# ZackHodari/morgana

Hardware: AMD Instinct MI355X
Metric: acoustic frames/sec (fwd+bwd+step), F0Model 600->1, batch 256x1000 (higher is better)
Workload: dtype bf16

## Files before the change

### morgana_amd/csrc/gemm_bf16_big.hip

```cpp
#include "common.h"
#include "phone_front.h"
#include "expand_reduce.h"

#include <type_traits>

typedef __bf16 bfv8 __attribute__((ext_vector_type(8)));
typedef __bf16 bfv4 __attribute__((ext_vector_type(4)));


#define MG_ZERO_ELEMS 16384
__device__ uint16_t g_zero_row[MG_ZERO_ELEMS];

__device__ __forceinline__ void glds16(const uint16_t* src, unsigned char* lds_wave_base) {
    const unsigned lds_off = (unsigned)(unsigned long long)((__attribute__((address_space(3))) unsigned char*)lds_wave_base);
    const unsigned lds_uni = __builtin_amdgcn_readfirstlane(lds_off);
    unsigned keep;
    asm volatile("s_mov_b32 %0, m0\n\ts_mov_b32 m0, %2\n\ts_nop 0\n\tglobal_load_lds_dwordx4 %1, off\n\ts_mov_b32 m0, %0"
                 : "=&s"(keep)
                 : "v"(src), "s"(lds_uni)
                 : "memory");
}


#define WAIT_VM_BARRIER(N) asm volatile("s_waitcnt vmcnt(" #N ")\n\ts_barrier" ::: "memory")
#define WAIT_LGKM_BARRIER() asm volatile("s_waitcnt lgkmcnt(0)\n\ts_barrier" ::: "memory")

MG_STAMP_DECL(g_stamps_nt);

#define NT_BIG_LDS(BN_) (((BN_) == 256 ? 4 : 6) * (256 * 64 + (BN_) * 64))
template <int BN, int EPI, int X3 = 0>
__device__ __forceinline__ void gemm_nt_big_body(unsigned char* __restrict__ smem, const unsigned block_id, const uint16_t* __restrict__ A,
                                                 int lda, const int32_t* __restrict__ rows, int64_t M, int K, const uint16_t* __restrict__ Bm,
                                                 int ldb, int N, const float* __restrict__ bias_in, const uint16_t* __restrict__ H, int ldh,
                                                 const int32_t* __restrict__ h_rows, void* __restrict__ Cv_in, int ldc, int tiles_m, int tiles_n,
                                                 int c_f32, float* __restrict__ colsum = nullptr, int wt = 0) {
    const float* bias = bias_in;
    void* Cv = Cv_in;
    constexpr int BM = 256;
    constexpr int WAVES_N = BN / 64;
    constexpr int WAVES_M = 8 / WAVES_N;
    constexpr int WM = BM / WAVES_M;
    constexpr int TM = WM / 32, TN = 2;
    constexpr int A_BYTES = BM * 64, B_BYTES = BN * 64;
    constexpr int STAGE = A_BYTES + B_BYTES;
    constexpr int GA = BM / 16 / 8;
    constexpr int GB = BN / 16 / 8;
    constexpr int NL = GA + GB;
    constexpr int NS = (BN == 256) ? 4 : 6;

    static_assert(NS * STAGE == NT_BIG_LDS(BN), "LDS size helper");

    unsigned tile_id = block_id;
    int my_pass = 0;
    if (X3 == 2) {
        const unsigned per_pass = (unsigned)((tiles_m + 7) / 8) * 8u * (unsigned)tiles_n;
        my_pass = (int)(block_id / per_pass);
        tile_id = block_id - (unsigned)my_pass * per_pass;
    }
    const int xcd = tile_id & 7, jj = tile_id >> 3;
    const int tile_n = jj % tiles_n;
    const int tile_m = (jj / tiles_n) * 8 + xcd;
    if (tile_m >= tiles_m) return;

    const int tid = threadIdx.x, lane = tid & 63;
    const int wave = __builtin_amdgcn_readfirstlane(tid >> 6);
#ifdef MG_STAMPS
    unsigned long long ts0, ts1 = 0, ts2, ts3, tr0, tr1, ta, tb, sum_wait = 0, sum_issue = 0;
    MG_STAMP(ts0);
    MG_STAMP_REAL(tr0);
#endif
    const int wm0 = (wave / WAVES_N) * WM, wn0 = (wave % WAVES_N) * 64;
    const int64_t m0 = (int64_t)tile_m * BM;
    const int n0 = tile_n * BN;
    const int n_kp = (K + 31) / 32;
    const int n_kt = X3 == 1 ? 3 * n_kp : n_kp;
    const int a_lo = lda >> 1, b_lo = ldb >> 1;
    if (X3 == 2) {
        if (my_pass > 0) bias = nullptr;
        Cv = reinterpret_cast<float*>(Cv) + (size_t)my_pass * (size_t)M * ldc;
    }

    const uint16_t* asrc[GA];
    const uint16_t* bsrc[GB];
#pragma unroll
    for (int i = 0; i < GA; ++i) {
        const int row = (wave * GA + i) * 16 + (lane >> 2);
        const int c = (lane & 3) ^ ((row >> 2) & 3);
        const int64_t m = m0 + row;
        const uint16_t* p = g_zero_row;
        if (m < M) {
            if (rows) {
                const int r = rows[m];
                if (r >= 0) p = A + (size_t)r * lda;
            } else {
                p = A + (size_t)m * lda;
            }
        }
        asrc[i] = p + c * 8;
    }
#pragma unroll
    for (int i = 0; i < GB; ++i) {
        const int row = (wave * GB + i) * 16 + (lane >> 2);
        const int c = (lane & 3) ^ ((row >> 2) & 3);
        const int n = n0 + row;
        bsrc[i] = (n < N ? Bm + (size_t)n * ldb : g_zero_row) + c * 8;
    }

    auto issue = [&](int kt) {
        unsigned char* st = smem + (kt % NS) * STAGE;
        int ka = kt * 32, kb = kt * 32;
        if (X3) {
            const int pass = X3 == 2 ? my_pass : kt % 3, w = (X3 == 2 ? kt : kt / 3) * 32;
            ka = w + (pass == 2 ? a_lo : 0);
            kb = w + (pass == 1 ? b_lo : 0);
        }
#pragma unroll
        for (int i = 0; i < GA; ++i) glds16(asrc[i] + ka, st + (wave * GA + i) * 1024);
#pragma unroll
        for (int i = 0; i < GB; ++i) glds16(bsrc[i] + kb, st + A_BYTES + (wave * GB + i) * 1024);
    };

    f32x16 acc[TM][TN];
#pragma unroll
    for (int i = 0; i < TM; ++i)
#pragma unroll
        for (int j = 0; j < TN; ++j)
#pragma unroll
            for (int r = 0; r < 16; ++r) acc[i][j][r] = 0.f;

    const int lr = lane & 31, lh = lane >> 5;
    int aoff[TM], boff[TN];
#pragma unroll
    for (int i = 0; i < TM; ++i) {
        const int row = wm0 + i * 32 + lr;
        aoff[i] = row * 64 + ((lh ^ ((row >> 2) & 3)) << 4);
    }
#pragma unroll
    for (int j = 0; j < TN; ++j) {
        const int row = wn0 + j * 32 + lr;
        boff[j] = A_BYTES + row * 64 + ((lh ^ ((row >> 2) & 3)) << 4);
    }

#pragma unroll
    for (int p = 0; p < NS - 1; ++p)
        if (p < n_kt) issue(p);
    for (int kt = 0; kt < n_kt; ++kt) {
        MG_STAMP(ta);
        {
            const int fly = min(n_kt - 1 - kt, NS - 2);
            if (NL == 4) {
                if (fly >= 2) WAIT_VM_BARRIER(8); else if (fly == 1) WAIT_VM_BARRIER(4); else WAIT_VM_BARRIER(0);
            } else if (NS == 4) {
                if (fly >= 2) WAIT_VM_BARRIER(6); else if (fly == 1) WAIT_VM_BARRIER(3); else WAIT_VM_BARRIER(0);
            } else {
                if (fly >= 4) WAIT_VM_BARRIER(12); else if (fly == 3) WAIT_VM_BARRIER(9); else if (fly == 2) WAIT_VM_BARRIER(6);
                else if (fly == 1) WAIT_VM_BARRIER(3); else WAIT_VM_BARRIER(0);
            }
        }
        MG_STAMP(tb);
        MG_STAMP_ADD(sum_wait, tb, ta);
#ifdef MG_STAMPS
        if (kt == 0) ts1 = tb;
#endif
        if (kt + NS - 1 < n_kt) issue(kt + NS - 1);
        MG_STAMP(ta);
        MG_STAMP_ADD(sum_issue, ta, tb);
        const unsigned char* st = smem + (kt % NS) * STAGE;
#pragma unroll
        for (int ks = 0; ks < 2; ++ks) {
            bfv8 a[TM], b[TN];
#pragma unroll
            for (int i = 0; i < TM; ++i) a[i] = *reinterpret_cast<const bfv8*>(st + (aoff[i] ^ (ks << 5)));
#pragma unroll
            for (int j = 0; j < TN; ++j) b[j] = *reinterpret_cast<const bfv8*>(st + (boff[j] ^ (ks << 5)));
#pragma unroll
            for (int i = 0; i < TM; ++i)
#pragma unroll
                for (int j = 0; j < TN; ++j) {
                    if (EPI_IS_GRAD(EPI)) acc[i][j] = mg_mfma_32x32x16(a[i], b[j], acc[i][j]);
                    else acc[i][j] = mg_mfma_32x32x16(b[j], a[i], acc[i][j]);
                }
        }
    }

#ifdef MG_STAMPS
    MG_STAMP(ts2);
#endif
    if (EPI_IS_GRAD(EPI)) {
        constexpr int STG_LD = 68;
        WAIT_LGKM_BARRIER();
        float* stg = reinterpret_cast<float*>(smem) + wave * 32 * STG_LD;
        float csum[8];
#pragma unroll
        for (int e = 0; e < 8; ++e) csum[e] = 0.f;
#pragma unroll
        for (int i = 0; i < TM; ++i) {
#pragma unroll
            for (int j = 0; j < TN; ++j)
#pragma unroll
                for (int r = 0; r < 16; ++r) stg[((r & 3) + 8 * (r >> 2) + 4 * lh) * STG_LD + j * 32 + lr] = acc[i][j][r];
#pragma unroll
            for (int it = 0; it < 4; ++it) {
                const int rl = it * 8 + (lane >> 3);
                const int cl = (lane & 7) * 8;
                const int64_t row = m0 + wm0 + i * 32 + rl;
                const int col = n0 + wn0 + cl;
                const f32x4 v0 = *reinterpret_cast<const f32x4*>(&stg[rl * STG_LD + cl]);
                const f32x4 v1 = *reinterpret_cast<const f32x4*>(&stg[rl * STG_LD + cl + 4]);
                if (row >= M) continue;
                const int64_t hrow = h_rows ? (int64_t)h_rows[row] : row;
                const bfv8 hv = *reinterpret_cast<const bfv8*>(H + (size_t)hrow * ldh + col);
                float v[8] = {v0.x, v0.y, v0.z, v0.w, v1.x, v1.y, v1.z, v1.w};
                if (X3) {
                    const bfv8 hl = *reinterpret_cast<const bfv8*>(H + (size_t)hrow * ldh + (ldh >> 1) + col);
                    bfv8 o_hi, o_lo;
#pragma unroll
                    for (int e = 0; e < 8; ++e) {
#pragma clang fp contract(off)
                        const float h = (float)hv[e] + (float)hl[e];
                        const float x = v[e] * h * (1.f - h);
                        csum[e] += x;
                        o_hi[e] = (__bf16)x;
                        o_lo[e] = (__bf16)(x - (float)o_hi[e]);
                    }
                    uint16_t* crow = reinterpret_cast<uint16_t*>(Cv) + (size_t)row * ldc + col;
                    mg_store16_sel(wt, crow, __builtin_bit_cast(mg_u32x4, o_hi));
                    mg_store16_sel(wt, crow + (ldc >> 1), __builtin_bit_cast(mg_u32x4, o_lo));
                    continue;
                }
#pragma unroll
                for (int e = 0; e < 8; ++e) v[e] = mg_epi_dact<EPI>(v[e], (float)hv[e]);
                if (c_f32) {
                    float* crow = reinterpret_cast<float*>(Cv) + (size_t)row * ldc + col;
                    *reinterpret_cast<f32x4*>(crow) = f32x4{v[0], v[1], v[2], v[3]};
                    *reinterpret_cast<f32x4*>(crow + 4) = f32x4{v[4], v[5], v[6], v[7]};
                } else {
                    bfv8 o;
#pragma unroll
                    for (int e = 0; e < 8; ++e) o[e] = (__bf16)v[e];
                    mg_store16_sel(wt, reinterpret_cast<uint16_t*>(Cv) + (size_t)row * ldc + col, __builtin_bit_cast(mg_u32x4, o));
                }
            }
        }
        if (X3 && colsum) {
#pragma unroll
            for (int e = 0; e < 8; ++e) {
                csum[e] += __shfl_xor(csum[e], 8, 64);
                csum[e] += __shfl_xor(csum[e], 16, 64);
                csum[e] += __shfl_xor(csum[e], 32, 64);
            }
            if (lane < 8) {
                float* dst = colsum + ((size_t)tile_m * WAVES_M + (wave / WAVES_N)) * N + n0 + wn0 + lane * 8;
                *reinterpret_cast<f32x4*>(dst) = f32x4{csum[0], csum[1], csum[2], csum[3]};
                *reinterpret_cast<f32x4*>(dst + 4) = f32x4{csum[4], csum[5], csum[6], csum[7]};
            }
        }
        return;
    }

    float bv[TN][16];
    if (!EPI_IS_GRAD(EPI)) {
#pragma unroll
        for (int j = 0; j < TN; ++j)
#pragma unroll
            for (int g = 0; g < 4; ++g)
#pragma unroll
                for (int e = 0; e < 4; ++e) bv[j][4 * g + e] = bias ? bias[n0 + wn0 + j * 32 + 8 * g + 4 * lh + e] : 0.f;
    }
    if (!c_f32) {
        constexpr int SP = 144;
        WAIT_LGKM_BARRIER();
        unsigned char* patch = smem + wave * (32 * SP);
        const int prow = lane >> 3, pchunk = lane & 7;
#pragma unroll
        for (int i = 0; i < TM; ++i) {
#pragma unroll
            for (int j = 0; j < TN; ++j)
#pragma unroll
                for (int g = 0; g < 4; ++g) {
                    float v[4];
#pragma unroll
                    for (int e = 0; e < 4; ++e) {
                        float x = acc[i][j][4 * g + e] + bv[j][4 * g + e];
                        x = mg_epi_act<EPI, true>(x);
                        v[e] = x;
                    }
                    typedef __bf16 bfv2 __attribute__((ext_vector_type(2)));
                    typedef unsigned int u32x2_t __attribute__((ext_vector_type(2)));
                    const u32x2_t pk = u32x2_t{__builtin_bit_cast(unsigned int, bfv2{(__bf16)v[0], (__bf16)v[1]}),
                                               __builtin_bit_cast(unsigned int, bfv2{(__bf16)v[2], (__bf16)v[3]})};
                    *reinterpret_cast<u32x2_t*>(patch + lr * SP + (j * 32 + 8 * g + 4 * lh) * 2) = pk;
                }
#pragma unroll
            for (int it = 0; it < 4; ++it) {
                typedef unsigned int u32x4_t __attribute__((ext_vector_type(4)));
                const int rl = it * 8 + prow;
                const u32x4_t o = *reinterpret_cast<const u32x4_t*>(patch + rl * SP + pchunk * 16);
                const int64_t m = m0 + wm0 + i * 32 + rl;
                if (m < M) *reinterpret_cast<u32x4_t*>(reinterpret_cast<uint16_t*>(Cv) + (size_t)m * ldc + n0 + wn0 + pchunk * 8) = o;
            }
        }
    } else
#pragma unroll
    for (int i = 0; i < TM; ++i) {
        const int64_t m = m0 + wm0 + i * 32 + lr;
        const bool live = m < M;
#pragma unroll
        for (int j = 0; j < TN; ++j) {
            if (!live) continue;
            float* crow = reinterpret_cast<float*>(Cv) + (size_t)m * ldc + n0 + wn0 + j * 32 + 4 * lh;
#pragma unroll
            for (int g = 0; g < 4; ++g) {
                float v[4];
#pragma unroll
                for (int e = 0; e < 4; ++e) {
                    float x = acc[i][j][4 * g + e] + bv[j][4 * g + e];
                    x = mg_epi_act<EPI, true>(x);
                    v[e] = x;
                }
                *reinterpret_cast<f32x4*>(crow + 8 * g) = f32x4{v[0], v[1], v[2], v[3]};
            }
        }
    }
#ifdef MG_STAMPS
    asm volatile("s_waitcnt vmcnt(0)" ::: "memory");
    MG_STAMP(ts3);
    MG_STAMP_REAL(tr1);
    const int sb = block_id;
    MG_STAMP_STORE(g_stamps_nt, sb, wave, lane, 0, ts0);
    MG_STAMP_STORE(g_stamps_nt, sb, wave, lane, 1, ts1);
    MG_STAMP_STORE(g_stamps_nt, sb, wave, lane, 2, ts2);
    MG_STAMP_STORE(g_stamps_nt, sb, wave, lane, 3, ts3);
    MG_STAMP_STORE(g_stamps_nt, sb, wave, lane, 4, tr0);
    MG_STAMP_STORE(g_stamps_nt, sb, wave, lane, 5, tr1);
    MG_STAMP_STORE(g_stamps_nt, sb, wave, lane, 6, sum_wait);
    MG_STAMP_STORE(g_stamps_nt, sb, wave, lane, 7, sum_issue);
#endif
}

template <int BN, int EPI, int X3 = 0>
__global__ __launch_bounds__(512) void gemm_nt_big_kernel(const uint16_t* __restrict__ A, int lda, const int32_t* __restrict__ rows,
                                                          int64_t M, int K, const uint16_t* __restrict__ Bm, int ldb, int N,
                                                          const float* __restrict__ bias, const uint16_t* __restrict__ H, int ldh,
                                                          const int32_t* __restrict__ h_rows, void* __restrict__ Cv, int ldc, int tiles_m,
                                                          int tiles_n, int c_f32) {
    __shared__ __attribute__((aligned(16))) unsigned char smem[NT_BIG_LDS(BN)];
    gemm_nt_big_body<BN, EPI, X3>(smem, blockIdx.x, A, lda, rows, M, K, Bm, ldb, N, bias, H, ldh, h_rows, Cv, ldc, tiles_m, tiles_n, c_f32);
}

#define NTP_MAX_TILES(BN_) ((BN_) == 256 ? 8 : 7)
__device__ uint16_t g_ntp_sink[64 * 8];
MG_STAMP_DECL(g_stamps_ntp);

#define WAIT_VM_LGKM_BARRIER(N) asm volatile("s_waitcnt vmcnt(" #N ") lgkmcnt(0)\n\ts_barrier" ::: "memory")
#define NTP_WAIT_CASE(N) case N: WAIT_VM_LGKM_BARRIER(N); break;

template <int BN, int BK, int MODE>
constexpr int ntp_lds_bytes() {
    constexpr int STAGE = 256 * BK * 2 + BN * BK * 2;
    constexpr int NS = (BK == 64) ? (BN == 256 ? 2 : 3) : ((BN == 256) ? 4 : 5);
    constexpr int PATCH = NS * STAGE + NTP_MAX_TILES(BN) * 256 * 4;
    constexpr bool kPatchInRing = MODE != 1 && STAGE >= 8 * 32 * 128;
    return PATCH + (kPatchInRing ? 0 : (MODE == 1 ? 8 * 32 * 64 : 8 * 32 * 128)) + BN * 4;
}

template <int BN, int EPI, bool STAG, int BK, int MODE = 0, int BMV = 256, int X3 = 0>
__device__ __forceinline__ void gemm_nt_persist_body(unsigned char* __restrict__ smem, const unsigned block_id, const unsigned n_blocks,
                                                     const uint16_t* __restrict__ A, int lda, const int32_t* __restrict__ rows, int64_t M,
                                                     int K, const uint16_t* __restrict__ Bm, int ldb, int N, const float* __restrict__ bias,
                                                     uint16_t* __restrict__ C, int ldc, int tiles_m, int tiles_n, int probe,
                                                     int wt = 0) {
    constexpr bool PIPE = MODE == 1, ROLE = MODE == 5, SPREAD = MODE == 2;
    constexpr int BM = 256;
    constexpr int WAVES_N = BN / 64;
    constexpr int WAVES_M = 8 / WAVES_N;
    static_assert(BMV == 256 || (BMV == 192 && BN == 256 && MODE == 0 && !STAG), "192-row tiles: the plain square form only");
    constexpr int WM = BMV / WAVES_M;
    constexpr int TM = WM / 32, TN = 2;
    constexpr int ROWB = BK * 2;
    constexpr int KS = BK / 16;
    constexpr int LPR = ROWB / 16;
    constexpr int RPP = 64 / LPR;
    constexpr bool NATIVE = X3 == 2;
    constexpr int A_BYTES = BM * ROWB, B_BYTES = BN * ROWB;
    constexpr int PLANE = A_BYTES + B_BYTES;
    constexpr int STAGE = NATIVE ? 2 * PLANE : PLANE;
    constexpr int GA = BM / RPP / 8;
    constexpr int GB = BN / RPP / 8;
    constexpr int NL = (GA + GB) * (NATIVE ? 2 : 1);
    constexpr int NS = NATIVE ? 2 : ((BK == 64) ? (BN == 256 ? 2 : 3) : ((BN == 256) ? 4 : 5));
    constexpr int NST = TM * 4 * (X3 ? 2 : 1);
    static_assert(!X3 || (MODE == 0 && !STAG && BN == 256 && (BK == 32 || X3 == 1)), "X3: the plain square form only (native: 32-deep)");
    constexpr int ROWTAB = NS * STAGE;
    constexpr int MAXT = NTP_MAX_TILES(BN);
    constexpr int PATCH = ROWTAB + MAXT * BM * 4;
    constexpr int SP = 128;
    static_assert(!PIPE || (BN == 256 && BK == 32 && !STAG), "PIPE: square tile, 32-deep stages, lockstep");
    constexpr bool kPatchInRing = !PIPE && STAGE >= 8 * 32 * SP;
    constexpr int SPP = 64;
    constexpr int BIAS_OFF = PATCH + (kPatchInRing ? 0 : (PIPE ? 8 * 32 * SPP : 8 * 32 * SP));
    constexpr int LDS_BYTES = BIAS_OFF + BN * 4;
    static_assert(LDS_BYTES <= 160 * 1024, "LDS budget");

    static_assert(LDS_BYTES == ntp_lds_bytes<BN, BK, MODE>(), "LDS size helper");
    int* rowtab = reinterpret_cast<int*>(smem + ROWTAB);

    const int tid = threadIdx.x, lane = tid & 63;
    const int wave = __builtin_amdgcn_readfirstlane(tid >> 6);
#ifdef MG_STAMPS
    unsigned long long ts0, ts1 = 0, ts2, ts3, tr0, tr1, ta, tb, sum_wait = 0, sum_epi = 0;
    MG_STAMP(ts0);
    MG_STAMP_REAL(tr0);
#endif
    const int wm0 = (wave / WAVES_N) * WM, wn0 = (wave % WAVES_N) * 64;
    const int n_kp = (K + BK - 1) / BK;
    const int n_kt = X3 == 1 ? 3 * n_kp : n_kp;
    const int a_lo = lda >> 1, b_lo = ldb >> 1;

    auto tile_of = [&](int i, int& tile_m, int& tile_n) {
        const int v = (int)(block_id + i * n_blocks);
        const int xcd = v & 7, jj = v >> 3;
        tile_n = jj % tiles_n;
        tile_m = (jj / tiles_n) * 8 + xcd;
    };
    int n_my = 0;
    for (int i = 0; i < MAXT; ++i) {
        int tm, tn;
        tile_of(i, tm, tn);
        if (tm < tiles_m) n_my = i + 1;
    }
    for (int e = tid; e < n_my * BM; e += 512) {
        int tm, tn;
        tile_of(e / BM, tm, tn);
        const int64_t m = (int64_t)tm * BMV + (e % BM);
        int r = -1;
        if (m < M && (e % BM) < BMV) r = rows ? rows[m] : (int)m;
        rowtab[e] = r;
    }
    __syncthreads();
    if (n_my == 0) return;

    auto swz = [](int row) { return BK == 32 ? ((row >> 2) & 3) : ((row >> 1) & 7); };
    const uint16_t* asrc[GA];
    const uint16_t* bsrc[GB];
    auto set_sources = [&](int i) {
        int tm, tn;
        tile_of(i, tm, tn);
#pragma unroll
        for (int g = 0; g < GA; ++g) {
            const int row = (wave * GA + g) * RPP + lane / LPR;
            const int c = (lane % LPR) ^ swz(row);
            const int r = rowtab[i * BM + row];
            asrc[g] = (r >= 0 ? A + (size_t)r * lda : g_zero_row) + c * 8;
        }
#pragma unroll
        for (int g = 0; g < GB; ++g) {
            const int row = (wave * GB + g) * RPP + lane / LPR;
            const int c = (lane % LPR) ^ swz(row);
            const int n = tn * BN + row;
            bsrc[g] = (n < N ? Bm + (size_t)n * ldb : g_zero_row) + c * 8;
        }
    };
    int i_t = 0, i_k = 0, i_s = 0, i_p = 0, i_w = 0;
    set_sources(0);
    auto issue_next = [&](int reps = 1) {
        if (i_t >= n_my) return;
        unsigned char* st = smem + i_s * STAGE;
        const int ka = X3 == 1 ? i_w * BK + (i_p == 2 ? a_lo : 0) : i_k * BK;
        const int kb = X3 == 1 ? i_w * BK + (i_p == 1 ? b_lo : 0) : i_k * BK;
        if (NATIVE) {
#pragma unroll
            for (int pl = 0; pl < 2; ++pl) {
#pragma unroll
                for (int g = 0; g < GA; ++g) glds16(asrc[g] + ka + pl * a_lo, st + pl * PLANE + (wave * GA + g) * 1024);
#pragma unroll
                for (int g = 0; g < GB; ++g) glds16(bsrc[g] + kb + pl * b_lo, st + pl * PLANE + A_BYTES + (wave * GB + g) * 1024);
            }
        } else
        for (int rep = 0; rep < reps; ++rep) {
#pragma unroll
        for (int g = 0; g < GA; ++g)
            if (!(probe & 1)) glds16(asrc[g] + ka, st + (wave * GA + g) * 1024);
#pragma unroll
        for (int g = 0; g < GB; ++g)
            if (!(probe & 2)) glds16(bsrc[g] + kb, st + A_BYTES + (wave * GB + g) * 1024);
        }
        i_s = (i_s + 1 == NS) ? 0 : i_s + 1;
        if (X3 == 1 && ++i_p == 3) {
            i_p = 0;
            ++i_w;
        }
        if (++i_k == n_kt) {
            i_k = 0;
            i_p = 0;
// ... 469 lines not shown
    const int tiles = (N / BNT) * KH;
    int tile, s;
    if (xcd_group) {
        tile = (block_id >> 3) % tiles;
        s = (block_id / (8 * tiles)) * 8 + (block_id & 7);
    } else {
        tile = block_id % tiles;
        s = block_id / tiles;
    }
    const int n0 = (tile / KH) * BNT;
    const int kh = tile % KH, k0 = kh * BKT;
    const int64_t m_lo = (int64_t)s * m_chunk;
    const int64_t m_hi = min(M, m_lo + (int64_t)m_chunk);
    const int n_rows = m_hi > m_lo ? (int)(m_hi - m_lo) : 0;

    for (int i = tid; i < m_chunk; i += 512) {
        int r = -1;
        if (i < n_rows) r = rows ? rows[m_lo + i] : (int)(m_lo + i);
        row_lds[i] = r;
        if (DYR) dyrow_lds[i] = i < n_rows ? dy_rows[m_lo + i] : -1;
    }
    __syncthreads();

    int y_row[NY], y_c[NY];
#pragma unroll
    for (int i = 0; i < NY; ++i) {
        const int byte = (wave * NY + i) * 1024 + lane * 16;
        y_row[i] = byte / PY;
        y_c[i] = ((byte % PY) >> 4) ^ ((y_row[i] & 3) << 2);
    }
    int x_row[NX], x_off[NX];
#pragma unroll
    for (int i = 0; i < NX; ++i) {
        const int byte = (wave * NX + i) * 1024 + lane * 16;
        x_row[i] = byte / PX;
        const int cpos = (byte % PX) >> 4;
        const int src = cpos ^ ((x_row[i] & 3) << 2);
        x_off[i] = src < XC ? k0 + src * 8 : -1;
    }

    const int n_steps1 = (n_rows + 31) / 32;
    auto issue = [&](int step_all) {
        unsigned char* st = smem + (step_all % NSTG) * SLOT;
        int step = step_all, y_plane = 0, a_plane = 0;
        if (NATIVE) {
#pragma unroll
            for (int pl = 0; pl < 2; ++pl) {
#pragma unroll
                for (int i = 0; i < NY; ++i) {
                    const int ml = step * 32 + y_row[i];
                    const uint16_t* p = (ml < n_rows) ? dY + (size_t)(m_lo + ml) * lddy + pl * (lddy >> 1) + n0 + y_c[i] * 8 : g_zero_row;
                    glds16(p, st + pl * STAGE + (wave * NY + i) * 1024);
                }
                int rn[NX];
#pragma unroll
                for (int i = 0; i < NX; ++i) rn[i] = row_lds[step * 32 + x_row[i]];
#pragma unroll
                for (int i = 0; i < NX; ++i) {
                    const uint16_t* p = (rn[i] >= 0 && x_off[i] >= 0) ? A + (size_t)rn[i] * lda + pl * (lda >> 1) + x_off[i] : g_zero_row;
                    glds16(p, st + pl * STAGE + Y_BYTES + (wave * NX + i) * 1024);
                }
            }
            return;
        }
        if (X3) {
            step = step_all / 3;
            const int pass = step_all - 3 * step;
            y_plane = pass == 1 ? (lddy >> 1) : 0;
            a_plane = pass == 2 ? (lda >> 1) : 0;
        }
#pragma unroll
        for (int i = 0; i < NY; ++i) {
            if (DYR) {
                const int ry = dyrow_lds[step * 32 + y_row[i]];
                const uint16_t* p = ry >= 0 ? dY + (size_t)ry * lddy + n0 + y_c[i] * 8 : g_zero_row;
                glds16(p, st + (wave * NY + i) * 1024);
            } else {
                const int ml = step * 32 + y_row[i];
                const uint16_t* p = (ml < n_rows) ? dY + (size_t)(m_lo + ml) * lddy + y_plane + n0 + y_c[i] * 8 : g_zero_row;
                glds16(p, st + (wave * NY + i) * 1024);
            }
        }
        int rr[NX];
#pragma unroll
        for (int i = 0; i < NX; ++i) rr[i] = row_lds[step * 32 + x_row[i]];
#pragma unroll
        for (int i = 0; i < NX; ++i) {
            const uint16_t* p = (rr[i] >= 0 && x_off[i] >= 0) ? A + (size_t)rr[i] * lda + a_plane + x_off[i] : g_zero_row;
            glds16(p, st + Y_BYTES + (wave * NX + i) * 1024);
        }
    };

    f32x16 acc[TNW][TKT];
#pragma unroll
    for (int i = 0; i < TNW; ++i)
#pragma unroll
        for (int j = 0; j < TKT; ++j)
#pragma unroll
            for (int r = 0; r < 16; ++r) acc[i][j][r] = 0.f;
    constexpr bool kExtraBias = (TKW == 8 || TKW == 4);
    const bool free_tile = !kExtraBias && K <= KH * BKT - 32;
    const bool bias_free = bslab != nullptr && free_tile && kh == KH - 1 && (wave % WK) == WK - 1;
    const bool bias_extra = bslab != nullptr && kExtraBias && kh == 0 && (wave % WK) == 0;
    const bool bias_valu = bslab != nullptr && !kExtraBias && !free_tile && kh == 0;
    f32x16 accb[kExtraBias ? TNW : 1];
#pragma unroll
    for (int i = 0; i < (kExtraBias ? TNW : 1); ++i)
#pragma unroll
        for (int r = 0; r < 16; ++r) accb[i][r] = 0.f;
    const __bf16 one_bf = (__bf16)1.0f;
    const bfv8 ones = bfv8{one_bf, one_bf, one_bf, one_bf, one_bf, one_bf, one_bf, one_bf};
    float bsum = 0.f;

    const int n_steps = X3 == 1 ? 3 * n_steps1 : n_steps1;
    const int li = lane & 15, g = lane >> 4;
    const int q = li >> 2, p4 = li & 3;
    const int cgrp = 16 * (g & 1) + 4 * p4;
    const int rbase = 8 * (g >> 1) + q;
    const int sw = q << 2;
    int yoff[TNW], xoff[TKT];
#pragma unroll
    for (int i = 0; i < TNW; ++i) {
        const int col = wn0 + i * 32 + cgrp;
        yoff[i] = rbase * PY + ((((col >> 3) ^ sw) << 4) | ((col & 7) << 1));
    }
#pragma unroll
    for (int j = 0; j < TKT; ++j) {
        const int col = wk0 + j * 32 + cgrp;
        xoff[j] = Y_BYTES + rbase * PX + ((((col >> 3) ^ sw) << 4) | ((col & 7) << 1));
    }

#pragma unroll
    for (int p = 0; p < NSTG - 1; ++p)
        if (p < n_steps) issue(p);
    for (int step = 0; step < n_steps; ++step) {
        MG_STAMP(ta);
        if (NATIVE) {
            WAIT_VM_BARRIER(0);
        } else if (NSTG == 4 && step + 2 < n_steps) {
            if (NLW == 4) WAIT_VM_BARRIER(8); else WAIT_VM_BARRIER(6);
        } else if (step + 1 < n_steps) {
            if (NLW == 6) WAIT_VM_BARRIER(6); else if (NLW == 5) WAIT_VM_BARRIER(5); else if (NLW == 4) WAIT_VM_BARRIER(4); else WAIT_VM_BARRIER(3);
        } else {
            WAIT_VM_BARRIER(0);
        }
        MG_STAMP(tb);
        MG_STAMP_ADD(sum_wait, tb, ta);
#ifdef MG_STAMPS
        if (step == 0) ts1 = tb;
#endif
        if (step + NSTG - 1 < n_steps) issue(step + NSTG - 1);
        MG_STAMP(ta);
        MG_STAMP_ADD(sum_issue, ta, tb);
        const unsigned char* st = smem + (step % NSTG) * SLOT;
        if constexpr (NATIVE) {
#pragma unroll
            for (int ks = 0; ks < 2; ++ks) {
                bfv8 a[2][TNW], b[2][TKT];
#pragma unroll
                for (int pl = 0; pl < 2; ++pl) {
#pragma unroll
                    for (int i = 0; i < TNW; ++i) {
                        const unsigned char* ad = st + pl * STAGE + yoff[i] + ks * 16 * PY;
                        const bfv4 lo = __builtin_amdgcn_ds_read_tr16_b64_v4bf16((__attribute__((address_space(3))) bfv4*)(ad));
                        const bfv4 hi = __builtin_amdgcn_ds_read_tr16_b64_v4bf16((__attribute__((address_space(3))) bfv4*)(ad + 4 * PY));
                        a[pl][i] = bfv8{lo[0], lo[1], lo[2], lo[3], hi[0], hi[1], hi[2], hi[3]};
                    }
#pragma unroll
                    for (int j = 0; j < TKT; ++j) {
                        const unsigned char* ad = st + pl * STAGE + xoff[j] + ks * 16 * PX;
                        const bfv4 lo = __builtin_amdgcn_ds_read_tr16_b64_v4bf16((__attribute__((address_space(3))) bfv4*)(ad));
                        const bfv4 hi = __builtin_amdgcn_ds_read_tr16_b64_v4bf16((__attribute__((address_space(3))) bfv4*)(ad + 4 * PX));
                        b[pl][j] = bfv8{lo[0], lo[1], lo[2], lo[3], hi[0], hi[1], hi[2], hi[3]};
                    }
                }
#pragma unroll
                for (int i = 0; i < TNW; ++i)
#pragma unroll
                    for (int j = 0; j < TKT; ++j) {
                        acc[i][j] = mg_mfma_32x32x16(a[0][i], b[0][j], acc[i][j]);
                        acc[i][j] = mg_mfma_32x32x16(a[1][i], b[0][j], acc[i][j]);
                        acc[i][j] = mg_mfma_32x32x16(a[0][i], b[1][j], acc[i][j]);
                    }
            }
            continue;
        }
#pragma unroll
        for (int ks = 0; ks < 2; ++ks) {
            bfv8 a[TNW], b[TKT];
#pragma unroll
            for (int i = 0; i < TNW; ++i) {
                const unsigned char* ad = st + yoff[i] + ks * 16 * PY;
                const bfv4 lo = __builtin_amdgcn_ds_read_tr16_b64_v4bf16((__attribute__((address_space(3))) bfv4*)(ad));
                const bfv4 hi = __builtin_amdgcn_ds_read_tr16_b64_v4bf16((__attribute__((address_space(3))) bfv4*)(ad + 4 * PY));
                a[i] = bfv8{lo[0], lo[1], lo[2], lo[3], hi[0], hi[1], hi[2], hi[3]};
            }
#pragma unroll
            for (int j = 0; j < TKT; ++j) {
                const unsigned char* ad = st + xoff[j] + ks * 16 * PX;
                const bfv4 lo = __builtin_amdgcn_ds_read_tr16_b64_v4bf16((__attribute__((address_space(3))) bfv4*)(ad));
                const bfv4 hi = __builtin_amdgcn_ds_read_tr16_b64_v4bf16((__attribute__((address_space(3))) bfv4*)(ad + 4 * PX));
                b[j] = bfv8{lo[0], lo[1], lo[2], lo[3], hi[0], hi[1], hi[2], hi[3]};
            }
            if (bias_free) b[TKT - 1] = ones;
#pragma unroll
            for (int i = 0; i < TNW; ++i)
#pragma unroll
                for (int j = 0; j < TKT; ++j) acc[i][j] = mg_mfma_32x32x16(a[i], b[j], acc[i][j]);
            if constexpr (kExtraBias) {
                if (bias_extra) {
#pragma unroll
                    for (int i = 0; i < TNW; ++i) accb[i] = mg_mfma_32x32x16(a[i], ones, accb[i]);
                }
            }
        }
        if (bias_valu && tid < BNT) {
#pragma unroll 8
            for (int r = 0; r < 32; ++r) {
                const int cpos = (tid >> 3) ^ ((r & 3) << 2);
                bsum += mg_bf2f(*reinterpret_cast<const uint16_t*>(st + r * PY + (cpos << 4) + ((tid & 7) << 1)));
            }
        }
    }

#ifdef MG_STAMPS
    MG_STAMP(ts2);
#endif
    const int lr = lane & 31, lh = lane >> 5;
    float* out = slab + (size_t)s * sstride;
#pragma unroll
    for (int i = 0; i < TNW; ++i) {
#pragma unroll
        for (int j = 0; j < TKT; ++j) {
            const int col = k0 + wk0 + j * 32 + lr;
            if (col >= K) continue;
#pragma unroll
            for (int r = 0; r < 16; ++r) {
                const int row = n0 + wn0 + i * 32 + (r & 3) + 8 * (r >> 2) + 4 * lh;
                if (row < N) mg_store_sel(WT, &out[(size_t)row * K + col], acc[i][j][r]);
            }
        }
    }
    if (bias_valu && tid < BNT && n0 + tid < N) mg_store_sel(WT, &bslab[(size_t)s * sstride + n0 + tid], bsum);
    if ((bias_free || bias_extra) && lr == 0) {
#pragma unroll
        for (int i = 0; i < TNW; ++i) {
#pragma unroll
            for (int r = 0; r < 16; ++r) {
                const int row = n0 + wn0 + i * 32 + (r & 3) + 8 * (r >> 2) + 4 * lh;
                const float v = bias_free ? acc[i][TKT - 1][r] : accb[kExtraBias ? i : 0][r];
                if (row < N) mg_store_sel(WT, &bslab[(size_t)s * sstride + row], v);
            }
        }
    }
#ifdef MG_STAMPS
    asm volatile("s_waitcnt vmcnt(0)" ::: "memory");
    MG_STAMP(ts3);
    MG_STAMP_REAL(tr1);
    const int sb = block_id;
    MG_STAMP_STORE(g_stamps_wg, sb, wave, lane, 0, ts0);
    MG_STAMP_STORE(g_stamps_wg, sb, wave, lane, 1, ts1);
    MG_STAMP_STORE(g_stamps_wg, sb, wave, lane, 2, ts2);
    MG_STAMP_STORE(g_stamps_wg, sb, wave, lane, 3, ts3);
    MG_STAMP_STORE(g_stamps_wg, sb, wave, lane, 4, tr0);
    MG_STAMP_STORE(g_stamps_wg, sb, wave, lane, 5, tr1);
    MG_STAMP_STORE(g_stamps_wg, sb, wave, lane, 6, sum_wait);
    MG_STAMP_STORE(g_stamps_wg, sb, wave, lane, 7, sum_issue);
#endif
}

template <int TKW, int NW = 1, int X3 = 0>
__global__ __launch_bounds__(512) void wgrad_big_kernel(const uint16_t* __restrict__ dY, int lddy, const uint16_t* __restrict__ A, int lda,
                                                        const int32_t* __restrict__ rows, int64_t M, int N, int K, int m_chunk,
                                                        float* __restrict__ slab, float* __restrict__ bslab, int64_t sstride, int xcd_group) {
    __shared__ __attribute__((aligned(16))) unsigned char smem[WG_BIG_LDS_NW(TKW, NW)];
    wgrad_big_body<TKW, false, NW, X3>(smem, blockIdx.x, dY, lddy, A, lda, rows, M, N, K, m_chunk, slab, bslab, sstride, xcd_group);
}

template <int TKW, int NW = 1>
__global__ __launch_bounds__(512) void wgrad_big_rows_kernel(const uint16_t* __restrict__ dY, int lddy, const int32_t* __restrict__ dy_rows,
                                                             const uint16_t* __restrict__ A, int lda, const int32_t* __restrict__ rows, int64_t M,
                                                             int N, int K, int m_chunk, float* __restrict__ slab, float* __restrict__ bslab,
                                                             int64_t sstride, int xcd_group) {
    __shared__ __attribute__((aligned(16))) unsigned char smem[WG_BIG_LDS_NW(TKW, NW) + WG_ROWS_MAX * 4];
    wgrad_big_body<TKW, true, NW>(smem, blockIdx.x, dY, lddy, A, lda, rows, M, N, K, m_chunk, slab, bslab, sstride, xcd_group, dy_rows);
}

template <int TKW, int BN, int X3 = 0>
__global__ __launch_bounds__(512) void wgrad_dgrad_pair_kernel(unsigned wg_blocks, const uint16_t* __restrict__ dY, int lddy,
                                                               const uint16_t* __restrict__ A, int lda, int64_t M, int N, int K, int m_chunk,
                                                               float* __restrict__ slab, float* __restrict__ bslab, int64_t sstride,
                                                               int xcd_group, const uint16_t* __restrict__ WT, int ldwt,
                                                               const uint16_t* __restrict__ H, int ldh, void* __restrict__ dX, int lddx,
                                                               int tiles_m, int tiles_n, unsigned nt_blocks, ExpandReduceArgs xr, int riders,
                                                               float* __restrict__ colsum, int wt) {
    constexpr int LDS = WG_BIG_LDS(TKW) > NT_BIG_LDS(BN) ? WG_BIG_LDS(TKW) : NT_BIG_LDS(BN);
    __shared__ __attribute__((aligned(16))) unsigned char smem[LDS];
    if (blockIdx.x < wg_blocks) {
        constexpr int WX3 = (X3 && WG_STAGES(TKW) == 4) ? 2 : X3;
        if (wt) wgrad_big_body<TKW, false, 1, WX3, true>(smem, blockIdx.x, dY, lddy, A, lda, nullptr, M, N, K, m_chunk, slab, bslab, sstride, xcd_group);
        else wgrad_big_body<TKW, false, 1, WX3, false>(smem, blockIdx.x, dY, lddy, A, lda, nullptr, M, N, K, m_chunk, slab, bslab, sstride, xcd_group);
    }
    else if (blockIdx.x < wg_blocks + nt_blocks)
        gemm_nt_big_body<BN, EPI_SIGMOID_GRAD, X3>(smem, blockIdx.x - wg_blocks, dY, lddy, nullptr, M, N, WT, ldwt, K, nullptr, H, ldh, nullptr, dX,
                                                   lddx, tiles_m, tiles_n, 0, colsum, wt);
    else
        mg_expand_reduce_rider<512>(xr, (int)(blockIdx.x - wg_blocks - nt_blocks), riders, smem);
}


static bool big16(const void* p) { return ((uintptr_t)p % 16) == 0; }

int mg_try_nt_big(const uint16_t* A, int lda, const int32_t* rows, int64_t M, int K, const uint16_t* Bm, int ldb, int N,
                  const float* bias, const uint16_t* H, int ldh, const int32_t* h_rows, void* C, int ldc, int c_f32, int epi,
                  hipStream_t st) {
    if (M < 2048 || lda % 64 != 0 || ldb % 64 != 0 || lda > MG_ZERO_ELEMS - 64 || ldb > MG_ZERO_ELEMS - 64) return 0;
    if (N % 128 != 0 || ldc < N || ldc % 8 != 0 || !big16(A) || !big16(Bm) || !big16(C)) return 0;
    if (EPI_IS_GRAD(epi) && (!H || ldh % 8 != 0 || ldh < N)) return 0;
    if (ldc != N || lda < (K + 63) / 64 * 64 || ldb < (K + 63) / 64 * 64) return 0;
    const int ab = g_mg_tuning[MG_TUNE_AB];
    if (ab == 98 && M < 32768) return 0;
    bool wide = (N % 256 == 0);
    if (wide && ab != 97 && (ab == 99 || mg_ceil_div(M, 256) * (N / 256) < 128)) wide = false;
    const int bn = wide ? 256 : 128;
    const int tiles_n = N / bn;
    const int64_t tiles_m = mg_ceil_div(M, 256);
    const int64_t blocks = mg_ceil_div(tiles_m, 8) * 8 * tiles_n;
    if (blocks >= 2147483647LL || tiles_m >= 2147483647LL) return 0;
    const int n_kt = (K + 31) / 32;
    if (!c_f32 && !EPI_IS_GRAD(epi) && n_kt >= 5 && M < 2147483647LL && 32 % tiles_n == 0 && g_mg_tuning[MG_TUNE_FORM] != 6) {
        int64_t g = 256;
        while (mg_ceil_div(blocks, g) > NTP_MAX_TILES(bn)) g += 256;
        if (g > blocks) g = mg_ceil_div(blocks, 8 * tiles_n) * 8 * tiles_n;
        dim3 pgrid((unsigned)g), pblock(512);
#define LAUNCH_NTP(BN_, EPI_, STAG_, BK_) hipLaunchKernelGGL((gemm_nt_persist_kernel<BN_, EPI_, STAG_, BK_>), pgrid, pblock, 0, st, A, lda, rows, M, K, Bm, ldb, N, bias, (uint16_t*)C, ldc, (int)tiles_m, tiles_n, probe)
        const bool deep = g_mg_tuning[MG_TUNE_FORM] != 3;
#ifdef MG_EXPERIMENTS
        const int form = (epi == EPI_BIAS || epi == EPI_BIAS_SIGMOID) ? g_mg_tuning[MG_TUNE_FORM] : 0;
        const int probe = form >= 256 ? form - 256 : form >= 32 ? form - 32 : 0;
        if (wide && (form == 5 || form == 11)) {
            const int pr = form == 11 ? 32 : 0;
            if (epi == EPI_BIAS) hipLaunchKernelGGL((gemm_nt_persist_kernel<256, EPI_BIAS, false, 32, 2>), pgrid, pblock, 0, st, A, lda, rows, M, K, Bm, ldb, N, bias, (uint16_t*)C, ldc, (int)tiles_m, tiles_n, pr);
            else hipLaunchKernelGGL((gemm_nt_persist_kernel<256, EPI_BIAS_SIGMOID, false, 32, 2>), pgrid, pblock, 0, st, A, lda, rows, M, K, Bm, ldb, N, bias, (uint16_t*)C, ldc, (int)tiles_m, tiles_n, pr);
            return 1;
        }
        if (wide && (form == 9 || form == 10 || form == 12 || form == 13)) {
            hipLaunchKernelGGL((gemm_nt_persist_kernel<256, EPI_BIAS_SIGMOID, false, 32, 5>), pgrid, pblock, 0, st, A, lda, rows, M, K, Bm, ldb, N, bias, (uint16_t*)C, ldc, (int)tiles_m, tiles_n, form == 9 ? 16 : form == 10 ? 24 : form == 12 ? 23 : 23 + 64);
            return 1;
        }
        if (wide && form == 2) {
            if (epi == EPI_BIAS) hipLaunchKernelGGL((gemm_nt_persist_kernel<256, EPI_BIAS, false, 32, 1>), pgrid, pblock, 0, st, A, lda, rows, M, K, Bm, ldb, N, bias, (uint16_t*)C, ldc, (int)tiles_m, tiles_n, probe);
            else hipLaunchKernelGGL((gemm_nt_persist_kernel<256, EPI_BIAS_SIGMOID, false, 32, 1>), pgrid, pblock, 0, st, A, lda, rows, M, K, Bm, ldb, N, bias, (uint16_t*)C, ldc, (int)tiles_m, tiles_n, probe);
            return 1;
        }
        if (wide && form == 4) {
            if (epi == EPI_BIAS) LAUNCH_NTP(256, EPI_BIAS, true, 32); else LAUNCH_NTP(256, EPI_BIAS_SIGMOID, true, 32);
            return 1;
        }
#else
        const int probe = 0;
#endif
#define NTP_WIDE(EPI_) LAUNCH_NTP(256, EPI_, false, 32)
#define NTP_DEEP(EPI_) LAUNCH_NTP(128, EPI_, false, 64)
#define NTP_HALF(EPI_) LAUNCH_NTP(128, EPI_, false, 32)
        if (wide) MG_SWITCH_FWD_EPI(epi, NTP_WIDE);
        else if (deep) MG_SWITCH_FWD_EPI(epi, NTP_DEEP);
        else MG_SWITCH_FWD_EPI(epi, NTP_HALF);
#undef NTP_WIDE
#undef NTP_DEEP
#undef NTP_HALF
#undef LAUNCH_NTP
        return 1;
    }
    dim3 grid((unsigned)blocks), block(512);
#define LAUNCH_NT(BN_, EPI_) hipLaunchKernelGGL((gemm_nt_big_kernel<BN_, EPI_>), grid, block, 0, st, A, lda, rows, M, K, Bm, ldb, N, bias, H, ldh, h_rows, C, ldc, (int)tiles_m, tiles_n, c_f32)
#define NT_WIDE(EPI_) LAUNCH_NT(256, EPI_)
#define NT_HALF(EPI_) LAUNCH_NT(128, EPI_)
    if (wide) {
        if (EPI_IS_GRAD(epi)) MG_SWITCH_GRAD_EPI(epi, NT_WIDE);
        else MG_SWITCH_FWD_EPI(epi, NT_WIDE);
    } else {
        if (EPI_IS_GRAD(epi)) MG_SWITCH_GRAD_EPI(epi, NT_HALF);
        else MG_SWITCH_FWD_EPI(epi, NT_HALF);
    }
#undef NT_WIDE
#undef NT_HALF
#undef LAUNCH_NT
    return 1;
}

static bool wgrad_ksplit(int64_t M, int N, int lda) {
    if (g_mg_tuning[MG_TUNE_AB] == 92) return false;
    if (lda == 640) return M <= 32768 && N / 128 >= 4;
    return lda == 512 && N == 128 && M <= 32768 && g_mg_tuning[MG_TUNE_AB] != 93;
}

int mg_wgrad_big_plan(int64_t M, int N, int K, int lda, int lddy, int* S_out, int* m_chunk_out) {
    if (M < 4096 || N % 128 != 0 || lddy < N || lddy % 8 != 0) return 0;
    if (!((lda == 640 && K > 512 && K <= 640) || (lda == 512 && K > 384 && K <= 512))) return 0;
    const int tiles_n = N / 128;
    int64_t S = mg_ceil_div(256, tiles_n);
    if (M <= 32768 && tiles_n >= 4) S = 192 / tiles_n;
    if (wgrad_ksplit(M, N, lda)) {
        if (lda == 640) S = 256 / (2 * tiles_n);
        else S = 48;
    }
    if (M <= 32768 && tiles_n == 1) S = 96;
    if (M > 32768 && tiles_n == 1) S = 192;
    bool one_round = false;
    if (M > 32768 && tiles_n > 1 && !wgrad_ksplit(M, N, lda) && (int64_t)mg_align_up((size_t)S, 8) * tiles_n > 256 && tiles_n <= 128) {
        S = 256 / tiles_n;
        one_round = true;
    }
    const int ts = g_mg_tuning[MG_TUNE_WGRAD_SPLITS];
    if (ts > 0 && ts < 1000) S = ts;
    if (ts > 1000 && ts < 2000 && tiles_n == 1) S = ts - 1000;
    if (ts > 2000 && tiles_n >= 4) S = ts - 2000;
    int64_t m_chunk = mg_align_up((size_t)mg_ceil_div(M, S), 32);
    while (m_chunk > WG_ROWS_MAX) {
        S *= 2;
        m_chunk = mg_align_up((size_t)mg_ceil_div(M, S), 32);
    }
    S = mg_ceil_div(M, m_chunk);
    if (!one_round) S = mg_align_up((size_t)S, 8);
    if (S > 65535) return 0;
    *S_out = (int)S;
    *m_chunk_out = (int)m_chunk;
    return 1;
}

int mg_launch_wgrad_big(const uint16_t* dY, int lddy, const uint16_t* A, int lda, const int32_t* rows, int64_t M, int N, int K,
                        int S, int m_chunk, float* slab, float* bslab, int64_t sstride, hipStream_t st, const int32_t* dy_rows, int x3) {
    if (x3) {
        if (dy_rows || rows || bslab) return 0;
        const int pa = lda / 2;
        const bool ks = wgrad_ksplit(M, N, pa);
        dim3 grid((unsigned)((N / 128) * (ks ? 2 : 1) * S)), block(512);
        const int xg = (S % 8 == 0) ? 1 : 0;
#define LAUNCH_WG3(TKW_, NW_, X3_) hipLaunchKernelGGL((wgrad_big_kernel<TKW_, NW_, X3_>), grid, block, 0, st, dY, lddy, A, lda, rows, M, N, K, m_chunk, slab, bslab, sstride, xg)
        const bool walks = g_mg_tuning[MG_TUNE_AB] == 90;
        if (!ks && pa == 512 && N % 256 == 0) { if (walks) LAUNCH_WG3(4, 2, 1); else LAUNCH_WG3(4, 2, 2); }
        else if (ks && pa == 512) { if (walks) LAUNCH_WG3(4, 1, 1); else LAUNCH_WG3(4, 1, 2); }
        else if (ks) { if (walks) LAUNCH_WG3(5, 1, 1); else LAUNCH_WG3(5, 1, 2); }
        else if (pa == 640 && N % 256 == 0) LAUNCH_WG3(5, 2, 1);
        else if (pa == 640) LAUNCH_WG3(10, 1, 1);
        else LAUNCH_WG3(8, 1, 1);
#undef LAUNCH_WG3
        return 1;
    }
    if (dy_rows) {
        if (lda != 512 || wgrad_ksplit(M, N, lda)) return 0;
        dim3 grid((unsigned)((N / 128) * S)), block(512);
        const int xg = g_mg_tuning[MG_TUNE_WGRAD_ORDER] == 2 && S % 8 == 0 ? 1 : 0;
        if (N % 256 == 0 && g_mg_tuning[MG_TUNE_AB] != 91)
            hipLaunchKernelGGL((wgrad_big_rows_kernel<4, 2>), grid, block, 0, st, dY, lddy, dy_rows, A, lda, rows, M, N, K, m_chunk, slab, bslab,
                               sstride, xg);
        else
            hipLaunchKernelGGL((wgrad_big_rows_kernel<8>), grid, block, 0, st, dY, lddy, dy_rows, A, lda, rows, M, N, K, m_chunk, slab, bslab,
                               sstride, xg);
        return 1;
    }
    const bool ksplit = wgrad_ksplit(M, N, lda);
    dim3 grid((unsigned)((N / 128) * (ksplit ? 2 : 1) * S)), block(512);
    int xcd_group = (rows == nullptr && S % 8 == 0) ? 1 : 0;
    if (g_mg_tuning[MG_TUNE_WGRAD_ORDER] == 1) xcd_group = 0;
    if (g_mg_tuning[MG_TUNE_WGRAD_ORDER] == 2 && S % 8 == 0) xcd_group = 1;
    if (!ksplit && lda == 512 && N % 256 == 0 && g_mg_tuning[MG_TUNE_AB] != 91)
        hipLaunchKernelGGL((wgrad_big_kernel<4, 2>), grid, block, 0, st, dY, lddy, A, lda, rows, M, N, K, m_chunk, slab, bslab, sstride, xcd_group);
    else if (ksplit && lda == 512)
        hipLaunchKernelGGL((wgrad_big_kernel<4>), grid, block, 0, st, dY, lddy, A, lda, rows, M, N, K, m_chunk, slab, bslab, sstride, xcd_group);
    else if (ksplit)
        hipLaunchKernelGGL((wgrad_big_kernel<5>), grid, block, 0, st, dY, lddy, A, lda, rows, M, N, K, m_chunk, slab, bslab, sstride, xcd_group);
    else if (lda == 640 && N % 256 == 0 && g_mg_tuning[MG_TUNE_AB] != 91)
        hipLaunchKernelGGL((wgrad_big_kernel<5, 2>), grid, block, 0, st, dY, lddy, A, lda, rows, M, N, K, m_chunk, slab, bslab, sstride, xcd_group);
    else if (lda == 640)
        hipLaunchKernelGGL((wgrad_big_kernel<10>), grid, block, 0, st, dY, lddy, A, lda, rows, M, N, K, m_chunk, slab, bslab, sstride, xcd_group);
    else
        hipLaunchKernelGGL((wgrad_big_kernel<8>), grid, block, 0, st, dY, lddy, A, lda, rows, M, N, K, m_chunk, slab, bslab, sstride, xcd_group);
    return 1;
}

int mg_launch_phone_front_gemm(const PhoneFrontArgs& pf, const uint16_t* A, int lda, int64_t M, int K, const uint16_t* Bm, int ldb, int N,
                               const float* bias, uint16_t* C, int ldc, int epi, hipStream_t st) {
    if (g_mg_tuning[MG_TUNE_AB] == 66 || g_mg_tuning[MG_TUNE_FORM] != 0) return 0;
    if (M < 2048 || M >= 2147483647LL || lda % 64 != 0 || ldb % 64 != 0 || lda > MG_ZERO_ELEMS - 64 || ldb > MG_ZERO_ELEMS - 64) return 0;
    if (N % 256 != 0 || ldc != N || !big16(A) || !big16(Bm) || !big16(C)) return 0;
    if (lda < (K + 63) / 64 * 64 || ldb < (K + 63) / 64 * 64 || (K + 31) / 32 < 5) return 0;
    if (epi != EPI_BIAS && epi != EPI_BIAS_SIGMOID) return 0;
    const int tiles_n = N / 256;
    if (32 % tiles_n != 0) return 0;
    constexpr int LDS_INTS = ntp_lds_bytes<256, 32, 0>() / 4;
    const int64_t wave_ints_need = phone_front_wave_ints(pf.B, pf.P, pf.T, pf.extra);
    const int wave_ints = (g_mg_tuning[MG_TUNE_AB] != 94 && 8 * wave_ints_need <= LDS_INTS) ? (int)wave_ints_need : 0;
    int bmv = 256;
    if (wave_ints > 0 && g_mg_tuning[MG_TUNE_AB] != 95 && mg_ceil_div(mg_ceil_div(M, 192), 8) * 8 * tiles_n <= 224) bmv = 192;
    const int64_t tiles_m = mg_ceil_div(M, bmv);
    const int64_t blocks = mg_ceil_div(tiles_m, 8) * 8 * tiles_n;
    if (blocks > 224) return 0;
    const int64_t g = mg_ceil_div(blocks, 8 * tiles_n) * 8 * tiles_n;
    const int side = (int)((256 - g) / 8 * 8);
    if (side < 32) return 0;
    if (phone_front_lds_ints(pf.B, pf.P, pf.T, pf.extra) > LDS_INTS) return 0;
    PhoneFrontArgs a = pf;
    a.lds_ints = LDS_INTS;
#ifdef MG_EXPERIMENTS
    if (g_mg_tuning[MG_TUNE_AB] == 67) a.lds_ints = 0;
    if (g_mg_tuning[MG_TUNE_AB] >= 70 && g_mg_tuning[MG_TUNE_AB] < 85) a.probe = g_mg_tuning[MG_TUNE_AB] - 70;
#endif
    dim3 grid((unsigned)(side + g)), block(512);
#define LAUNCH_PFG(EPI_, BMV_, BK_)                                                                                                             \
    hipLaunchKernelGGL((phone_front_gemm_kernel<EPI_, BMV_, 0, BK_>), grid, block, 0, st, (unsigned)side, wave_ints, a, A, lda, M, K, Bm, ldb, N, bias, C, \
                       ldc, (int)tiles_m, tiles_n, wt)
    const int wt = (mg_wt_mask() & MG_WT_FWD) ? 1 : 0;
    const bool deep64 = g_mg_tuning[MG_TUNE_AB] == 88 && lda % 64 == 0 && ldb % 64 == 0;
    if (epi == EPI_BIAS) {
        if (bmv == 192) { if (deep64) LAUNCH_PFG(EPI_BIAS, 192, 64); else LAUNCH_PFG(EPI_BIAS, 192, 32); }
        else { if (deep64) LAUNCH_PFG(EPI_BIAS, 256, 64); else LAUNCH_PFG(EPI_BIAS, 256, 32); }
    } else {
        if (bmv == 192) { if (deep64) LAUNCH_PFG(EPI_BIAS_SIGMOID, 192, 64); else LAUNCH_PFG(EPI_BIAS_SIGMOID, 192, 32); }
        else { if (deep64) LAUNCH_PFG(EPI_BIAS_SIGMOID, 256, 64); else LAUNCH_PFG(EPI_BIAS_SIGMOID, 256, 32); }
    }
#undef LAUNCH_PFG
    return 1;
}

int mg_launch_wgrad_dgrad_pair(const uint16_t* dY, int lddy, const uint16_t* A, int lda, int64_t M, int N, int K, const uint16_t* WT, int ldwt,
                               uint16_t* dX, int lddx, float* slab, int64_t sstride, size_t slab_floats, int* S_out, hipStream_t st,
                               const ExpandReduceArgs* rider, int x3, float* colsum) {
    if (g_mg_tuning[MG_TUNE_AB] == 65) return 0;
    int S = 0, m_chunk = 0;
    const int pl = x3 ? 2 : 1;
    if (x3 && (lddy % 2 || lda % 2 || ldwt % 2 || lddx % 2 || !colsum)) return 0;
    const int lda_p = lda / pl, lddy_p = lddy / pl, ldwt_p = ldwt / pl;
    if (N != 128 || K != 512 || lda_p != 512 || lddx != pl * K || mg_wgrad_big_plan(M, N, K, lda_p, lddy_p, &S, &m_chunk) <= 0) return 0;
    if (lddy_p % 64 != 0 || ldwt_p % 64 != 0 || lddy > MG_ZERO_ELEMS - 64 || ldwt > MG_ZERO_ELEMS - 64 || lddy_p < 128 || ldwt_p < 128) return 0;
    if (!big16(dY) || !big16(A) || !big16(WT) || !big16(dX)) return 0;
    const int tiles_n = K / 256;
    const int64_t tiles_m = mg_ceil_div(M, 256);
    const bool ksplit = wgrad_ksplit(M, N, lda_p);
    const int kt = ksplit ? 2 : 1;
    auto fits = [&](int S_, int chunk_) {
        const int64_t s_real = mg_ceil_div(M, chunk_);
        for (int x = 0; x < 8; ++x) {
            const int64_t nt_x = (tiles_m > x ? mg_ceil_div(tiles_m - x, 8) : 0) * tiles_n;
            int64_t wg_x = 0;
            for (int b = x; b < S_; b += 8) wg_x += b < s_real ? kt : 0;
            if (nt_x + wg_x > 32) return false;
        }
        return true;
    };
    bool found = false;
    for (int cand = S; cand >= 48 / kt && !found; cand -= 8) {
        const int chunk_ = cand == S ? m_chunk : (int)mg_align_up((size_t)mg_ceil_div(M, cand), 32);
        if (chunk_ > WG_ROWS_MAX) break;
        const int S_ = (int)mg_align_up((size_t)mg_ceil_div(M, chunk_), 8);
        if (S_ > S || !fits(S_, chunk_)) continue;
        found = true;
        S = S_;
        m_chunk = chunk_;
    }
    if (!found) return 0;
    if ((size_t)S * (size_t)sstride > slab_floats) return 0;
    const unsigned nt_blocks = (unsigned)(mg_ceil_div(tiles_m, 8) * 8 * tiles_n);
    ExpandReduceArgs xr{};
    int riders = 0;
    if (rider) {
        xr = *rider;
        const int64_t by_frames = mg_ceil_div(xr.M, 2048), by_chunks = mg_ceil_div(mg_ceil_div(xr.n, 16) - xr.first_chunk, 2);
        riders = (int)(by_frames > by_chunks ? by_frames : by_chunks);
        if (riders < 1) riders = 1;
        if (riders > 1024) riders = 1024;
    }
    const int wt = (mg_wt_mask() & MG_WT_PAIR) ? 1 : 0;
    if (x3) {
        if (ksplit)
            hipLaunchKernelGGL((wgrad_dgrad_pair_kernel<4, 256, 1>), dim3((unsigned)(2 * S) + nt_blocks + riders), dim3(512), 0, st, (unsigned)(2 * S),
                               dY, lddy, A, lda, M, N, K, m_chunk, slab, (float*)nullptr, sstride, 1, WT, ldwt, A, lda, (void*)dX, lddx, (int)tiles_m,
                               tiles_n, nt_blocks, xr, riders, colsum, wt);
        else
            hipLaunchKernelGGL((wgrad_dgrad_pair_kernel<8, 256, 1>), dim3((unsigned)S + nt_blocks + riders), dim3(512), 0, st, (unsigned)S, dY, lddy,
                               A, lda, M, N, K, m_chunk, slab, (float*)nullptr, sstride, 1, WT, ldwt, A, lda, (void*)dX, lddx, (int)tiles_m, tiles_n,
                               nt_blocks, xr, riders, colsum, wt);
        *S_out = S;
        return 1;
    }
    if (ksplit)
        hipLaunchKernelGGL((wgrad_dgrad_pair_kernel<4, 256>), dim3((unsigned)(2 * S) + nt_blocks + riders), dim3(512), 0, st, (unsigned)(2 * S), dY,
                           lddy, A, lda, M, N, K, m_chunk, slab, slab + (int64_t)N * K, sstride, 1, WT, ldwt, A, lda, (void*)dX, lddx, (int)tiles_m,
                           tiles_n, nt_blocks, xr, riders, (float*)nullptr, wt);
    else
        hipLaunchKernelGGL((wgrad_dgrad_pair_kernel<8, 256>), dim3((unsigned)S + nt_blocks + riders), dim3(512), 0, st, (unsigned)S, dY, lddy, A, lda,
                           M, N, K, m_chunk, slab, slab + (int64_t)N * K, sstride, 1, WT, ldwt, A, lda, (void*)dX, lddx, (int)tiles_m, tiles_n,
                           nt_blocks, xr, riders, (float*)nullptr, wt);
    *S_out = S;
    return 1;
}

int mg_launch_nt_persist_x3(const PhoneFrontArgs* pf, const uint16_t* A, int lda, int64_t M, int K, const uint16_t* Bm, int ldb, int N,
                            const float* bias, uint16_t* C, int ldc, int epi, hipStream_t st, int* front_rode) {
    if (front_rode) *front_rode = 0;
    if (M < 1 || M >= 2147483647LL || lda % 128 != 0 || ldb % 128 != 0 || lda > MG_ZERO_ELEMS - 64 || ldb > MG_ZERO_ELEMS - 64) return 0;
    const int pa = lda / 2, pb = ldb / 2;
    if (N % 256 != 0 || ldc != 2 * N || !big16(A) || !big16(Bm) || !big16(C)) return 0;
    if (pa < (K + 63) / 64 * 64 || pb < (K + 63) / 64 * 64 || (K + 31) / 32 < 2) return 0;
    if (epi != EPI_BIAS && epi != EPI_BIAS_SIGMOID) return 0;
    const int tiles_n = N / 256;
    if (32 % tiles_n != 0) return 0;
// ... 99 lines not shown
```

Baseline: 2.540 billion.

## Prefetch activation-gradient H tile before main loop and buffer-store grad epilogue

In the NT GEMM body with a gradient epilogue, the H (activation) values are now loaded into registers before the K-loop, so their latency overlaps the MFMA work instead of stalling the epilogue. The epilogue also gets a new path that uses bounds-checked raw buffer stores, which drops the per-row M check and the column-sum accumulation. The fused wgrad/dgrad pair kernel opts out through a new template flag. This costs extra VGPRs held across the main loop, which may lower occupancy, and the new fast path skips colsum, so it depends on colsum not being needed in the standalone kernel.

```diff
diff --git a/morgana_amd/csrc/gemm_bf16_big.hip b/morgana_amd/csrc/gemm_bf16_big.hip
--- a/morgana_amd/csrc/gemm_bf16_big.hip
+++ b/morgana_amd/csrc/gemm_bf16_big.hip
@@ -28,7 +28,7 @@
 MG_STAMP_DECL(g_stamps_nt);
 
 #define NT_BIG_LDS(BN_) (((BN_) == 256 ? 4 : 6) * (256 * 64 + (BN_) * 64))
-template <int BN, int EPI, int X3 = 0>
+template <int BN, int EPI, int X3 = 0, bool AHEAD = true>
 __device__ __forceinline__ void gemm_nt_big_body(unsigned char* __restrict__ smem, const unsigned block_id, const uint16_t* __restrict__ A,
                                                  int lda, const int32_t* __restrict__ rows, int64_t M, int K, const uint16_t* __restrict__ Bm,
                                                  int ldb, int N, const float* __restrict__ bias_in, const uint16_t* __restrict__ H, int ldh,
@@ -106,6 +106,30 @@
         bsrc[i] = (n < N ? Bm + (size_t)n * ldb : g_zero_row) + c * 8;
     }
 
+    constexpr bool H_AHEAD = EPI_IS_GRAD(EPI) && !X3 && AHEAD;
+    bfv8 hq[H_AHEAD ? TM : 1][4];
+    if (H_AHEAD) {
+        const int col = n0 + wn0 + (lane & 7) * 8;
+        int64_t hrow[TM][4];
+#pragma unroll
+        for (int i = 0; i < TM; ++i)
+#pragma unroll
+            for (int it = 0; it < 4; ++it) {
+                const int64_t row = m0 + wm0 + i * 32 + it * 8 + (lane >> 3);
+                hrow[i][it] = row < M ? row : M - 1;
+            }
+        if (h_rows) {
+#pragma unroll
+            for (int i = 0; i < TM; ++i)
+#pragma unroll
+                for (int it = 0; it < 4; ++it) hrow[i][it] = (int64_t)h_rows[hrow[i][it]];
+        }
+#pragma unroll
+        for (int i = 0; i < TM; ++i)
+#pragma unroll
+            for (int it = 0; it < 4; ++it) hq[H_AHEAD ? i : 0][it] = *reinterpret_cast<const bfv8*>(H + (size_t)hrow[i][it] * ldh + col);
+    }
+
     auto issue = [&](int kt) {
         unsigned char* st = smem + (kt % NS) * STAGE;
         int ka = kt * 32, kb = kt * 32;
@@ -188,8 +212,57 @@
 #endif
     if (EPI_IS_GRAD(EPI)) {
         constexpr int STG_LD = 68;
+        if (H_AHEAD) __builtin_amdgcn_s_waitcnt(0x0F70);
         WAIT_LGKM_BARRIER();
         float* stg = reinterpret_cast<float*>(smem) + wave * 32 * STG_LD;
+        const int rows_live = (int)(M - m0 < BM ? M - m0 : BM);
+        auto store_rows = [&](auto wt_form, auto f32_form) {
+            constexpr bool F32 = decltype(f32_form)::value;
+            constexpr int AUX = decltype(wt_form)::value ? 16 : 0;
+            constexpr int ES = F32 ? 4 : 2;
+            const auto rs = __builtin_amdgcn_make_buffer_rsrc(reinterpret_cast<unsigned char*>(Cv) + (size_t)m0 * ldc * ES, 0, rows_live * ldc * ES,
+                                                              0x00020000);
+            int ln = lane;
+            asm volatile("" : "+v"(ln));
+            const int lr = ln & 31, lh = ln >> 5;
+            const int cl = (ln & 7) * 8;
+            const int col = n0 + wn0 + cl;
+#pragma unroll
+            for (int i = 0; i < TM; ++i) {
+#pragma unroll
+                for (int j = 0; j < TN; ++j)
+#pragma unroll
+                    for (int r = 0; r < 16; ++r) stg[((r & 3) + 8 * (r >> 2) + 4 * lh) * STG_LD + j * 32 + lr] = acc[i][j][r];
+#pragma unroll
+                for (int it = 0; it < 4; ++it) {
+                    const int rl = it * 8 + (ln >> 3);
+                    const int off = ((wm0 + i * 32 + rl) * ldc + col) * ES;
+                    const f32x4 v0 = *reinterpret_cast<const f32x4*>(&stg[rl * STG_LD + cl]);
+                    const f32x4 v1 = *reinterpret_cast<const f32x4*>(&stg[rl * STG_LD + cl + 4]);
+                    bfv8 hv = hq[H_AHEAD ? i : 0][it];
+                    asm volatile("" : "+v"(hv));
+                    float v[8] = {v0.x, v0.y, v0.z, v0.w, v1.x, v1.y, v1.z, v1.w};
+#pragma unroll
+                    for (int e = 0; e < 8; ++e) v[e] = mg_epi_dact<EPI>(v[e], (float)hv[e]);
+                    if (F32) {
+                        __builtin_amdgcn_raw_buffer_store_b128(__builtin_bit_cast(mg_u32x4, f32x4{v[0], v[1], v[2], v[3]}), rs, off, 0, AUX);
+                        __builtin_amdgcn_raw_buffer_store_b128(__builtin_bit_cast(mg_u32x4, f32x4{v[4], v[5], v[6], v[7]}), rs, off + 16, 0, AUX);
+                    } else {
+                        bfv8 o;
+#pragma unroll
+                        for (int e = 0; e < 8; ++e) o[e] = (__bf16)v[e];
+                        __builtin_amdgcn_raw_buffer_store_b128(__builtin_bit_cast(mg_u32x4, o), rs, off, 0, AUX);
+                    }
+                    __builtin_amdgcn_sched_barrier(0);
+                }
+            }
+        };
+        if (H_AHEAD) {
+            if (c_f32) store_rows(std::false_type{}, std::true_type{});
+            else if (wt) store_rows(std::true_type{}, std::false_type{});
+            else store_rows(std::false_type{}, std::false_type{});
+            return;
+        }
         float csum[8];
 #pragma unroll
         for (int e = 0; e < 8; ++e) csum[e] = 0.f;
@@ -1265,7 +1338,7 @@
         else wgrad_big_body<TKW, false, 1, WX3, false>(smem, blockIdx.x, dY, lddy, A, lda, nullptr, M, N, K, m_chunk, slab, bslab, sstride, xcd_group);
     }
     else if (blockIdx.x < wg_blocks + nt_blocks)
-        gemm_nt_big_body<BN, EPI_SIGMOID_GRAD, X3>(smem, blockIdx.x - wg_blocks, dY, lddy, nullptr, M, N, WT, ldwt, K, nullptr, H, ldh, nullptr, dX,
+        gemm_nt_big_body<BN, EPI_SIGMOID_GRAD, X3, false>(smem, blockIdx.x - wg_blocks, dY, lddy, nullptr, M, N, WT, ldwt, K, nullptr, H, ldh, nullptr, dX,
                                                    lddx, tiles_m, tiles_n, 0, colsum, wt);
     else
         mg_expand_reduce_rider<512>(xr, (int)(blockIdx.x - wg_blocks - nt_blocks), riders, smem);
```

Result: no change. 2.534 billion (-0.2%).
